# chrism0dwk/covid19uk

Measured on AMD Instinct MI355X. Metric: posterior samples/sec, 380-LAD UK SEIR, higher is better.
Workload: dtype f64; 1 GPU; uk380: M=380 LADs x T=365 days, P=750 parameters; chains_per_gpu=8, chains_total=8, sweep=HMC(16 leapfrogs) + 5 x [S->E move, E->I move, S->E occult, E->I occult], draws_recorded=theta + events[M,T,3] (uint16 counts) + kernel results per sweep, parallelism=chains sharded over 1 GPU(s), no data-path collective

## Files before the change

covid19uk_amd/csrc/handoff.h:

```cpp
#pragma once
#include <hip/hip_runtime.h>

template <typename T> __device__ __forceinline__ T ld_l2(const T *p) { return __hip_atomic_load(p, __ATOMIC_RELAXED, __HIP_MEMORY_SCOPE_AGENT); }
template <typename T, typename V> __device__ __forceinline__ void st_l2(T *p, V v) { __hip_atomic_store(p, v, __ATOMIC_RELAXED, __HIP_MEMORY_SCOPE_AGENT); }
template <typename T, typename V> __device__ __forceinline__ T add_l2(T *p, V v) { return __hip_atomic_fetch_add(p, v, __ATOMIC_RELAXED, __HIP_MEMORY_SCOPE_AGENT); }
template <typename T, typename V> __device__ __forceinline__ T min_l2(T *p, V v) { return __hip_atomic_fetch_min(p, v, __ATOMIC_RELAXED, __HIP_MEMORY_SCOPE_AGENT); }
template <typename T, typename V> __device__ __forceinline__ T max_l2(T *p, V v) { return __hip_atomic_fetch_max(p, v, __ATOMIC_RELAXED, __HIP_MEMORY_SCOPE_AGENT); }

__device__ __forceinline__ bool hs_all(bool ok) { return __builtin_amdgcn_ballot_w64(!ok) == 0ull; }

constexpr int HS_LIMIT = 1 << 22;
constexpr int HS_LIMIT_LEAP = 1 << 21;
constexpr int HS_LIMIT_LL = 1 << 19;
constexpr int HS_LIMIT_ROLES = 4000;
constexpr int HS_CHECK = 256;
constexpr int HS_CHECK_LL = 64;
enum HsCount { HS_CALLER, HS_THREAD0, HS_LANE0, HS_NONE };

template <int SLEEP, int CHECK, int LIMIT, int WHO, int FIRST = SLEEP, int PRIO = -1, typename Ready, typename C = unsigned>
__device__ __forceinline__ bool hs_wait(Ready ready, C *cnt = nullptr, bool backoff = false) {
    static_assert((CHECK & (CHECK - 1)) == 0, "CHECK: a power of two, or 0");
    int spins = 0;
    bool gave_up = false;
    while (!ready()) {
// ... 86 lines not shown
    constexpr int NW = (NDW + 1) / 2;
    const uint4 *pp[1] = {src + min(lane, NW - 1)};
    u32x4 x[1];
    ll_wait<1, 1, HS_CHECK, HS_LIMIT>(pp, seq, late, x);
    if (lane < NW) {
        dst[2 * lane] = (int)x[0].x;
        if (2 * lane + 1 < NDW) dst[2 * lane + 1] = (int)x[0].z;
    }
}

__device__ __forceinline__ void pair_sums_store(uint4 *dst, double th, double cn, unsigned seq) {
    ll_store(dst, th, seq);
    ll_store(dst + 1, cn, seq);
}
__device__ __forceinline__ void pair_sums_wait(const uint4 *src, unsigned seq, unsigned *late, double &th, double &cn) {
    const uint4 *pp[2] = {src, src + 1};
    u32x4 x[2];
    ll_wait<2, 1, HS_CHECK, HS_LIMIT>(pp, seq, late, x);
    th = ll_value(x[0]);
    cn = ll_value(x[1]);
}

__device__ __forceinline__ unsigned pair_token(unsigned sweep, int lidx) { return (sweep * 64u + (unsigned)lidx + 1u) & 0x7fffffffu; }
```

covid19uk_amd/csrc/moves_kernel.h:

```cpp
#pragma once
#include "handoff.h"
#include "sampler_kernels.h"

namespace seir {

#ifdef SEIR_STAMPS
#ifndef SEIR_STAMP_SLOT
#define SEIR_STAMP_SLOT 1
#endif
#define MSTAMP(i) do { if (threadIdx.x == 0 && stamp_on) ((unsigned long long *)(stamp_hs + 16))[i] = __builtin_amdgcn_s_memrealtime(); } while (0)
#else
#define MSTAMP(i) do {} while (0)
#endif

#ifdef PAIR_STAMPS
#define QSTAMP(slot_, step_, i_) do { if (threadIdx.x == 0 && (b_stamp) == 0 && (step_) < 12 && (slot_) < 27) \
    ch.leap_st[((size_t)(slot_) * 12 + (step_)) * 16 + (i_)] = __builtin_amdgcn_s_memrealtime(); } while (0)
#else
#define QSTAMP(slot_, step_, i_) do {} while (0)
#endif

constexpr int MVB = 512;
constexpr int MVW = MVB / WAVE;
constexpr int MVU = 4;
// ... 26 lines not shown

__device__ __forceinline__ void mv_sum2(double &a, double &b2, double *sh) {
    a = wave_sum(a); b2 = wave_sum(b2);
    const int lane = threadIdx.x & 63, wave = threadIdx.x >> 6;
    lds_barrier();
    if (lane == 0) { sh[wave * 2] = a; sh[wave * 2 + 1] = b2; }
    lds_barrier();
    double x = 0.0, y = 0.0;
#pragma unroll
    for (int j = 0; j < MVW; ++j) { x += sh[j * 2]; y += sh[j * 2 + 1]; }
    a = x; b2 = y;
}

struct MvLds {
    const int *rt;
    int *rg;
#ifdef SEIR_STAMPS
    double *stamp_hs; bool stamp_on;
#endif
};

__device__ __forceinline__ double mv_log(double x, const double2 *ltab) { return x == 1.0 ? 0.0 : fast_log(x, ltab); }

__device__ inline void mv_draw(const SamplerCfg &s, const Chains &ch, int b, MoveSpec spec, MvShared &sm, int T) {
    Move &mv = sm.mv;
    const int tid = threadIdx.x;
    if (tid >= 2 * MMAX && tid != 64) return;
    const RngKey key = rng_key(s, ch, b);
    const uint32_t stream = RS_MOVE_BASE + (uint32_t)(spec.scan * 4 + spec.slot);
    if (tid < 2 * MMAX) rng_uniform2(key, stream, (uint32_t)tid, sm.u[tid][0], sm.u[tid][1]);
    if (tid == 64) {
        mv.valid = (s.disable_mask >> (1 + spec.slot)) & 1 ? 0 : 1;
        mv.n = 0; mv.tgt = spec.tgt; mv.kind = spec.kind; mv.slot = spec.slot;
        mv.logq = 0.0; mv.any_dI = 0; mv.LO = T; mv.HI = -1;
        for (int j = 0; j < MMAX; ++j) { mv.tm[j] = mv.tt[j] = mv.tdt[j] = mv.tx[j] = 0; mv.b[j] = -1; sm.pend_valid[j] = -1; }
        double ua, ub;
        rng_uniform2(key, stream, 15u, ua, ub);
        mv.logu = cold_log(ua);
    }
}

__device__ __forceinline__ int wv_popc(unsigned long long m) { return __builtin_popcountll(m); }
__device__ __forceinline__ int wv_kth_bit(unsigned long long mask, int k, int lane) {
    const int below = (int)__builtin_amdgcn_mbcnt_hi((unsigned)(mask >> 32), __builtin_amdgcn_mbcnt_lo((unsigned)mask, 0u));
    const bool me = ((mask >> lane) & 1ull) != 0ull && below == k;
    return (int)__builtin_ctzll(__builtin_amdgcn_ballot_w64(me));
}
constexpr int WV_MCH = 6;
struct HotRows {
    unsigned long long mask[WV_MCH];
    int H;
// ... 568 lines not shown
                *prt += dk;
                if (ra + rb != 0) *prg += ra + rb;
            }
        }
        __syncthreads();
    }
}

__device__ __forceinline__ void mv_trace(const SamplerCfg &s, const Chains &ch, int b, const Move &mv, int acc,
                                         unsigned tr_slot, double lp) {
    if (tr_slot < (unsigned)s.cap) {
        double *tr = ch.tr_mv + (((size_t)tr_slot * s.B + b) * 4 + mv.slot) * NMVTR;
        tr[0] = (double)acc;
        tr[1] = lp;
        for (int j = 0; j < MMAX; ++j) {
            tr[2 + j] = mv.tm[j]; tr[2 + MMAX + j] = mv.tt[j];
            tr[2 + 2 * MMAX + j] = mv.tdt[j]; tr[2 + 3 * MMAX + j] = mv.tx[j];
        }
    }
}

__device__ __forceinline__ void mv_own_rows_to_down(const Dims &d, const Consts &c, const Work &w, int b, const Move &mv,
                                                    double psi, const double2 *ltab, const Move *fp, double *red,
                                                    double *od) {
    double dth = 0.0, dcn = 0.0;
    if (mv.valid && mv.n > 0) own_rows_delta<MVB>(d, c, w, b, mv, psi, 0, d.M, ltab, dth, dcn, fp);
    mv_sum2(dth, dcn, red);
    if (threadIdx.x == 0) {
        od[0] = dth;
        od[1] = dcn;
    }
}

struct PairNote {
    int ok;
    int n, rows[MMAX];
};
static_assert(sizeof(PairNote) == (2 + MMAX) * sizeof(int), "k_move_pair writes the note as 2 + MMAX ints");

__device__ __forceinline__ void move_copy_l2(Move *dst, const Move *src, int t0) {
    const int i = (int)threadIdx.x - t0;
    if (i >= 0 && i < MOVE_DW) reinterpret_cast<int *>(dst)[i] = ld_l2(reinterpret_cast<const int *>(src) + i);
}
__device__ __forceinline__ void wait_token(const unsigned *p_, unsigned token, unsigned *late) {
    hs_wait<1, HS_CHECK, HS_LIMIT, HS_CALLER>([&] { return ld_l2(p_) == token; }, late);
}
__device__ __forceinline__ unsigned wait_token_flag(const unsigned *p_, unsigned token, unsigned *late) {
    unsigned v;
    hs_wait<1, HS_CHECK, HS_LIMIT, HS_CALLER>([&] { return ((v = ld_l2(p_)) & 0x7fffffffu) == token; }, late);
    return v >> 31;
}
static_assert((MOVE_DW + 1) / 2 <= 32, "Chains::llmv holds 32 words per descriptor");
template <bool SOLO, typename TT>
// ... 233 lines not shown
                const int t = t0 + j * WAVE + lane;
                const bool in = t < d.Tp;
                k0[j] = in ? w.K[0][q0 + t] : 0;
                k1[j] = in ? w.K[1][q0 + t] : 0;
                k2[j] = in ? w.K[2][q0 + t] : 0;
            }
#pragma unroll
            for (int j = 0; j < 4; ++j) {
                const int t = t0 + j * WAVE + lane;
                if (t < d.T) {
                    if (s.ev16) {
                        if ((unsigned)(k0[j] | k1[j] | k2[j]) > 0xffffu) ch.ev_overflow[0] = 1u;
                        out16[t * 3 + 0] = (unsigned short)k0[j]; out16[t * 3 + 1] = (unsigned short)k1[j];
                        out16[t * 3 + 2] = (unsigned short)k2[j];
                    } else {
                        out[t * 3 + 0] = k0[j]; out[t * 3 + 1] = k1[j]; out[t * 3 + 2] = k2[j];
                    }
                }
            }
        }
    }
}

template <int NCH, bool SOLO>
__device__ __forceinline__ void pair_step(const Dims &d, const Consts &c, const Work &w, const SamplerCfg &s, const Chains &ch,
                                          MoveSpec se, MoveSpec next, MoveSpec se_next, int have_prev, int have_pre, int pbuf,
                                          int lidx, int dbg, int nband, int nroles, int slot, int b, int fin = 0,
                                          unsigned sweep0 = 0u, int lprev = 0, unsigned tslot = TRACE_NOT_RECORDED) {
    extern __shared__ __attribute__((aligned(16))) int dyn_i[];
    __shared__ MvShared sm_se, sm_nx;
    __shared__ Move pendA, pendB;
    __shared__ PairNote note;
    __shared__ double pre_down[2], s_down[4], s_dsum[2];
    __shared__ double2 ltab[LDSTAB_N];
    __shared__ int s_sel, s_acc_se, s_conf, s_late, s_late2, s_use_pre, s_trans;
    int tid = threadIdx.x;
    asm volatile("" : "+v"(tid));
    asm volatile("" : "+s"(b));
    const int b_stamp = b - d.b0;
    (void)b_stamp;
    QSTAMP(slot, lidx, 0);
    if (slot >= nroles) {
        if (nband == 0) return;
        if (fin) {
            pair_band_finish(d, c, w, s, ch, b, slot - nroles, nband, pair_token(sweep0, lidx), tslot, fin & 2);
            return;
        }
        const unsigned tok = pair_token(ch.sweep[b], lidx);
        const bool r1 = next.kind >= 0 && nroles >= 2, r2 = se_next.kind >= 0 && nroles == 3;
        if ((d.M + nband - 1) / nband > 2 * MVW)
            pair_band_block<SOLO, 4>(d, c, w, s, ch, b, slot - nroles, nband, tok, r1, r2, pbuf ^ 1, slot, lidx);
        else
            pair_band_block<SOLO, 2>(d, c, w, s, ch, b, slot - nroles, nband, tok, r1, r2, pbuf ^ 1, slot, lidx);
        return;
    }
    const int role = slot == nroles - 1 ? 0 : slot + 1;
    const int M = d.M, T = d.T;
    const bool do_se = role == 0 && se.kind >= 0, do_nx = next.kind >= 0, do_pre = se_next.kind >= 0 && nroles == 3;
    if (role == 1 && !do_nx) return;
    if (role == 2 && !do_pre) return;
#ifdef SEIR_STAMPS
    double *stamp_hs = ch.hs + (size_t)b * NHS;
    const bool stamp_on = do_se && b == 0 && se.slot == (SEIR_STAMP_SLOT & 2) && se.scan == 0;
#define PSTAMP(i) do { if (threadIdx.x == 0 && stamp_on) ((unsigned long long *)(stamp_hs + 16))[i] = __builtin_amdgcn_s_memrealtime(); } while (0)
#ifndef SEIR_STAMP_ROLE
#define SEIR_STAMP_ROLE 1
#endif
    const bool rstamp_on = role == SEIR_STAMP_ROLE && b == 0 && se.slot == (SEIR_STAMP_SLOT & 2) && se.scan == 0;
#ifdef SEIR_STAMP_PROPOSE
#define RSTAMP(i) do { if (threadIdx.x == 0 && rstamp_on) ((unsigned long long *)(stamp_hs + 16))[(i) + 4] = __builtin_amdgcn_s_memrealtime(); } while (0)
#undef PSTAMP
#define PSTAMP(i) do {} while (0)
#else
#define RSTAMP(i) do { if (threadIdx.x == 0 && rstamp_on) ((unsigned long long *)(stamp_hs + 16))[i] = __builtin_amdgcn_s_memrealtime(); } while (0)
#endif
#else
#define PSTAMP(i) do {} while (0)
#define RSTAMP(i) do {} while (0)
#endif
    PSTAMP(0);
    RSTAMP(8);
    const bool pre_ok = M <= PRE_RT * MVB;
    const MoveSpec &mine = role == 2 ? se_next : next;
    int pre_se[PRE_RT], pre_nx[PRE_RT];
    mv_prefetch_rows(d, w, s, b, se, do_se && pre_ok, pre_se);
    mv_prefetch_rows(d, w, s, b, mine, (role == 2 || do_nx) && pre_ok, pre_nx);
    const unsigned token = pair_token(ch.sweep[b], lidx);
    double dth0 = 0.0, dcn0 = 0.0;
    int ld_i = 0;
    double ld_d = 0.0;
    if (have_prev) {
        if (tid >= 64 && tid < 64 + MOVE_DW) ld_i = reinterpret_cast<const int *>(ch.mv + (size_t)pbuf * s.B + b)[tid - 64];
        if (tid >= 128 && tid < 128 + MOVE_DW) ld_i = reinterpret_cast<const int *>(ch.mvfix + (size_t)pbuf * s.B + b)[tid - 128];
        if (tid == 192) ld_i = ch.mvsel[(size_t)pbuf * s.B + b];
        if (tid >= 196 && tid < 200) ld_d = ch.Down[(((size_t)pbuf * 2 + ((tid - 196) >> 1)) * s.B + b) * 2 + ((tid - 196) & 1)];
        if (!SOLO) {
            if (tid < s.nrb_d) {
                dth0 = ch.Dpart[((size_t)b * s.nrb_d + tid) * 2];
                dcn0 = ch.Dpart[((size_t)b * s.nrb_d + tid) * 2 + 1];
            }
            for (int i = tid + MVB; i < s.nrb_d; i += MVB) {
                dth0 += ch.Dpart[((size_t)b * s.nrb_d + i) * 2];
                dcn0 += ch.Dpart[((size_t)b * s.nrb_d + i) * 2 + 1];
            }
        }
    }
    constexpr int DW0 = SOLO ? MVB - WAVE : 0;
    if (SOLO && have_prev) {
        static_assert(MVB >= 253, "one thread per band workgroup (plan_sweep: 3 + nband <= 256)");
        const bool few = s.nrb_d <= WAVE;
        const int i0 = few ? tid - DW0 : tid;
        if (few ? tid >= DW0 : (tid & ~(WAVE - 1)) < s.nrb_d) {
            const uint4 *src = ch.llD + (((size_t)pbuf * s.B + b) * s.nrb_d + min(i0, s.nrb_d - 1)) * 2;
            double th, cn;
            pair_sums_wait(src, pair_token(ch.sweep[b], lprev), ch.late + ch.late_fatal + b, th, cn);
            if (i0 < s.nrb_d) { dth0 = th; dcn0 = cn; }
#ifdef PAIR_STAMPS
            if (tid == DW0 && b_stamp == 0 && lidx < 12) ch.leap_st[((size_t)slot * 12 + lidx) * 16 + 7] = __builtin_amdgcn_s_memrealtime();
#endif
        }
    }
    const bool pre_avail = do_se && have_pre;
    if (pre_avail) {
        if (tid >= 256 && tid < 256 + MOVE_DW) ld_i = reinterpret_cast<const int *>(ch.mvs + (size_t)pbuf * s.B + b)[tid - 256];
        if (tid >= 320 && tid < 320 + 2 + MMAX) ld_i = reinterpret_cast<const int *>(ch.prev + (size_t)pbuf * s.B + b)[tid - 320];
        if (tid == 328 || tid == 329) ld_d = ch.DownS[((size_t)pbuf * s.B + b) * 2 + (tid - 328)];
    }
    static_assert(MOVE_DW <= 64 && 2 + MMAX <= 8, "the entry loads of pair_step: disjoint thread ranges");
    double hs_th = 0.0, hs_cn = 0.0, psi = 0.0;
    unsigned tr_slot = 0xffffffffu;
    double2 ld_t = make_double2(0.0, 0.0);
    if (tid < LDSTAB_N) ld_t = c.logtab[tid];
    if (role == 0 && tid == 0) {
        const double *hs = ch.hs + (size_t)b * NHS;
        hs_th = hs[HS_LP_THETA]; hs_cn = hs[HS_LP_CONST];
        tr_slot = SOLO ? tslot : chain_trace_slot(s, ch, ch.sweep[b]);
    }
    psi = w.scal[(size_t)b * NSCAL + SC_PSI];
    QSTAMP(slot, lidx, 6);
    if (do_se && !pre_avail) mv_draw(s, ch, b, se, sm_se, T);
    if (role != 0 || do_nx) mv_draw(s, ch, b, mine, sm_nx, T);
    QSTAMP(slot, lidx, 14);
    if (have_prev) {
        if (tid >= 64 && tid < 64 + MOVE_DW) reinterpret_cast<int *>(&pendA)[tid - 64] = ld_i;
        if (tid >= 128 && tid < 128 + MOVE_DW) reinterpret_cast<int *>(&pendB)[tid - 128] = ld_i;
        if (tid == 192) s_sel = ld_i;
        if (tid >= 196 && tid < 200) s_down[tid - 196] = ld_d;
    }
    if (pre_avail) {
        if (tid >= 256 && tid < 256 + MOVE_DW) reinterpret_cast<int *>(&sm_se.mv)[tid - 256] = ld_i;
        if (tid >= 320 && tid < 320 + 2 + MMAX) reinterpret_cast<int *>(&note)[tid - 320] = ld_i;
        if (tid == 328 || tid == 329) pre_down[tid - 328] = ld_d;
    }
    if (tid < LDSTAB_N) ltab[tid] = ld_t;
    if (have_prev && s.nrb_d <= WAVE && tid >= DW0 && tid < DW0 + WAVE) {
        const double a = wave_sum(dth0), a2 = wave_sum(dcn0);
        if (tid == DW0) { s_dsum[0] = 0.0 + a; s_dsum[1] = 0.0 + a2; }
    }
    if (role != 0) {
        asm volatile("s_waitcnt vmcnt(0)" ::: "memory");
        QSTAMP(slot, lidx, 12);
        __syncthreads();
        QSTAMP(slot, lidx, 13);
        const int late_bit = role == 1 ? 1 : 4, absent_bit = role == 1 ? 2 : 8;
// ... 15 lines not shown
        pendp = &pend;
        if (s.nrb_d <= WAVE) {
            dth0 = s_dsum[0]; dcn0 = s_dsum[1];
        } else {
            mv_sum2(dth0, dcn0, sm_nx.dred);
        }
        dth0 += s_down[s_sel ? 2 : 0];
        dcn0 += s_down[s_sel ? 3 : 1];
        const double ratio = dth0 + dcn0 + pend.logq;
        pend_acc = pend.valid && pend.logu < ratio;
    }
    if (role != 0) {
        const Move *fix = (pend_acc && pendp->tgt == mine.tgt) ? pendp : nullptr;
        RSTAMP(9);
#if defined(SEIR_STAMPS) && defined(SEIR_STAMP_PROPOSE)
        L.stamp_hs = stamp_hs; L.stamp_on = rstamp_on;
#endif
        QSTAMP(slot, lidx, 1);
        mv_rows_to_lds(d, w, s, b, mine, pre_ok, pre_nx, fix, L, rtl);
        mv_propose<NCH>(d, w, s, ch, b, mine, sm_nx, L, ltab);
        QSTAMP(slot, lidx, 2);
        RSTAMP(10);
        Move *out = (role == 1 ? ch.mv : ch.mvs) + (size_t)(pbuf ^ 1) * s.B + b;
        move_copy(out, &sm_nx.mv, MVB - WAVE);
        if (nband > 0 && role == 1 && tid >= MVB - WAVE)
            move_store_ll<MOVE_DW>(ch.llmv + ((size_t)(pbuf ^ 1) * s.B + b) * 32, reinterpret_cast<const int *>(&sm_nx.mv), tid - (MVB - WAVE),
                                   token);
        const Move *fpp = (pend_acc && pendp->any_dI) ? pendp : nullptr;
        double *od = role == 1 ? ch.Down + (((size_t)(pbuf ^ 1) * 2 + 0) * s.B + b) * 2
                               : ch.DownS + ((size_t)(pbuf ^ 1) * s.B + b) * 2;
        mv_own_rows_to_down(d, c, w, b, sm_nx.mv, psi, ltab, fpp, sm_nx.dred, od);
        QSTAMP(slot, lidx, 3);
        RSTAMP(11);
        if (nband > 0) {
            __syncthreads();
            if (tid == 0)
                st_l2(ch.done + (size_t)b * 2 * TAIL_STRIDE + role, token);
        }
        return;
    }
    if (!have_prev && tid == 64) {
        ch.fpend[b].valid = 0;
        if (nband > 0) {
            asm volatile("s_waitcnt vmcnt(0)" ::: "memory");
            st_l2(ch.done + (size_t)b * 2 * TAIL_STRIDE + 4, token);
        }
    }
    bool late = false, late2 = false;
    auto wait_roles = [&]() {
        if (tid == 0) {
            const bool l1 = do_nx && hs_wait<2, 0, HS_LIMIT_ROLES, HS_NONE>([&] { return ld_l2(ch.hand + b) == token; });
            const bool l2 = do_pre && hs_wait<2, 0, HS_LIMIT_ROLES, HS_NONE>([&] { return ld_l2(ch.hand2 + b) == token; });
            s_late = l1; s_late2 = l2;
            if (l1 || l2) ch.late[b] += 1;
// ... 33 lines not shown
            st_l2(ch.done + (size_t)b * 2 * TAIL_STRIDE + 5, token);
    }
    bool se_acc = false;
    if (do_se) {
        const Move *fpp = (pend_acc && pendp->any_dI) ? pendp : nullptr;
        if (tid == 0) {
            int use = pre_avail && note.ok;
            if (use) {
                const Move &mv = sm_se.mv;
                for (int i = 0; i < mv.n; ++i) {
                    for (int j = 0; j < note.n; ++j) use &= mv.m[i] != note.rows[j];
                    if (pend_acc)
                        for (int j = 0; j < pendp->n; ++j) use &= mv.m[i] != pendp->m[j];
                }
            }
            s_use_pre = use;
        }
        lds_barrier();
        const bool use_pre = s_use_pre != 0;
        double dth = 0.0, dcn = 0.0;
        if (!use_pre) {
            if (pre_avail) {
                lds_barrier();
                mv_draw(s, ch, b, se, sm_se, T);
            }
            mv_rows_to_lds(d, w, s, b, se, pre_ok, pre_se, nullptr, L, rtl);
            PSTAMP(2);
            mv_propose<NCH>(d, w, s, ch, b, se, sm_se, L, ltab);
            PSTAMP(3);
        }
        const Move &mv = sm_se.mv;
        if (use_pre && fpp == nullptr) {
            dth = pre_down[0]; dcn = pre_down[1];
        } else {
            if (mv.valid && mv.n > 0) own_rows_delta<MVB>(d, c, w, b, mv, psi, 0, M, ltab, dth, dcn, fpp);
            PSTAMP(4);
            mv_sum2(dth, dcn, sm_se.dred);
        }
        if (tid == 0) {
            const double ratio = dth + dcn + mv.logq;
            s_acc_se = (mv.valid && mv.logu < ratio) ? 1 : 0;
        }
        lds_barrier();
        se_acc = s_acc_se != 0;
        if (se_acc && !waited) { wait_roles(); waited = true; }
        if (tid == 0) s_trans = 0;
        if (se_acc) mv_apply_rows(d, w, s, b, mv, &s_trans);
// ... 39 lines not shown
            move_copy(ch.mvfix + (size_t)(pbuf ^ 1) * s.B + b, &sm_nx.mv, MVB - WAVE);
            const Move *fpp = (pend_acc && pendp->any_dI) ? pendp : nullptr;
            mv_own_rows_to_down(d, c, w, b, sm_nx.mv, psi, ltab, fpp, sm_nx.dred,
                                ch.Down + (((size_t)(pbuf ^ 1) * 2 + 1) * s.B + b) * 2);
        }
        PSTAMP(7);
        QSTAMP(slot, lidx, 3);
    }
    if (do_pre && tid == 0) {
        int *nt = reinterpret_cast<int *>(ch.prev + (size_t)(pbuf ^ 1) * s.B + b);
        const int n_pend = pend_acc ? pendp->n : 0, n_se = se_acc ? sm_se.mv.n : 0;
        const bool se_keeps = !se_acc || (((s_trans & (se_next.kind == 0 ? 1 : 2)) == 0) && n_pend + n_se <= MMAX);
        nt[0] = (se_keeps && !(waited && late2)) ? 1 : 0;
        nt[1] = n_pend + (se_keeps ? n_se : 0);
#pragma unroll
        for (int j = 0; j < MMAX; ++j) {
            int row = -1;
            if (j < n_pend) row = pendp->m[j];
            else if (se_keeps && j - n_pend < n_se) row = sm_se.mv.m[j - n_pend];
            nt[2 + j] = row;
        }
    }
    if (nband > 0) {
        __syncthreads();
        if (tid == 0)
            st_l2(ch.done + (size_t)b * 2 * TAIL_STRIDE + 0, token | ((do_nx && s_conf) ? 0x80000000u : 0u));
    }
}

template <int NCH>
__global__ __launch_bounds__(MVB) void k_move_pair(Dims d, Consts c, Work w, SamplerCfg s, Chains ch, MoveSpec se,
                                                   MoveSpec next, MoveSpec se_next, int have_prev, int have_pre,
                                                   int pbuf, int nbk, int lidx, int dbg, int nband) {
    debug_skew(d);
    const int nroles = (int)gridDim.x / nbk - nband, slot = (int)blockIdx.x / nbk;
    const int b = d.b0 + (int)blockIdx.x - slot * nbk;
    if (d.nlive > 0 && (int)blockIdx.x - slot * nbk >= d.nlive) return;
    pair_step<NCH, false>(d, c, w, s, ch, se, next, se_next, have_prev, have_pre, pbuf, lidx, dbg, nband, nroles, slot, b);
    const int b_stamp = b - d.b0;
    (void)b_stamp;
    QSTAMP(slot, lidx, 8);
}

constexpr int PBAR_STRIDE = 64;
__device__ __forceinline__ void pair_chain_barrier(const Chains &ch, int b, unsigned target, int b_stamp = 0, int st_slot = 0,
                                                   int st_step = 0) {
    asm volatile("s_waitcnt vmcnt(0)" ::: "memory");
    __syncthreads();
    QSTAMP(st_slot, st_step, 10);
    if (threadIdx.x == 0) {
        unsigned *cnt = ch.pbar + (size_t)b * PBAR_STRIDE;
        const unsigned old = add_l2(cnt, 1u);
        __builtin_amdgcn_fence(__ATOMIC_ACQUIRE, "agent");
#ifndef PBAR_SLEEP
#define PBAR_SLEEP 1
#endif
        if (old + 1u != target)
            hs_wait<PBAR_SLEEP, HS_CHECK, HS_LIMIT, HS_CALLER>([&] { return (int)(ld_l2(cnt) - target) >= 0; }, ch.late + ch.late_fatal + b);
        asm volatile("s_waitcnt vmcnt(0)" ::: "memory");
    }
    QSTAMP(st_slot, st_step, 11);
    __syncthreads();
}

__device__ __forceinline__ void pair_band_next_step() {
    __syncthreads();
    if (threadIdx.x == 0) {
        __builtin_amdgcn_fence(__ATOMIC_ACQUIRE, "agent");
        asm volatile("s_waitcnt vmcnt(0)" ::: "memory");
    }
    __syncthreads();
}

constexpr int PAIR_DBG_DELAYS = 16 | 32 | 64 | 128;
__device__ __forceinline__ void pair_debug_delay(int dbg, int slot, int nroles, int pair, int b) {
    const bool band = slot >= nroles, role0 = slot == nroles - 1;
    bool on = ((dbg & 16) && band) || ((dbg & 32) && role0) || ((dbg & 64) && !band && !role0);
    if (dbg & 128) {
        unsigned h = (unsigned)slot * 0x9e3779b1u ^ (unsigned)pair * 0x85ebca6bu ^ (unsigned)b * 0xc2b2ae35u;
        h ^= h >> 15; h *= 0x2c1b3c6du; h ^= h >> 12;
        on = on || h % 3u == 0u;
    }
    if (on)
        for (int i = 0; i < 9; ++i) __builtin_amdgcn_s_sleep(127);
}

template <int NCH>
__global__ __launch_bounds__(MVB) void k_move_pairs(Dims d, Consts c, Work w, SamplerCfg s, Chains ch, int npairs, int pre_on,
                                                    int nbk, int dbg, int nband, unsigned pbase, int fin) {
    debug_skew(d);
    const int nroles = (int)gridDim.x / nbk - nband, slot = (int)blockIdx.x / nbk;
    const int b = d.b0 + (int)blockIdx.x - slot * nbk;
    if (d.nlive > 0 && (int)blockIdx.x - slot * nbk >= d.nlive) return;
    const MoveSpec none{-1, 0, 0, 0};
    const unsigned sweep0 = ch.sweep[b];
    const unsigned tslot = chain_trace_slot(s, ch, sweep0);
    for (int pair = 0; pair <= npairs; ++pair) {
        const bool closing = pair == npairs;
        const int scan = pair >> 1, half = pair & 1, nh = half ^ 1, nscan = scan + half;
        const bool pre = pre_on && pair + 1 < npairs;
        const MoveSpec se = closing ? none : MoveSpec{half, 0, 2 * half, scan};
        const MoveSpec nx = closing ? MoveSpec{-2, 0, 0, 0} : MoveSpec{half, 1, 2 * half + 1, scan};
        const MoveSpec se_next = pre ? MoveSpec{nh, 0, 2 * nh, nscan} : none;
        if (dbg & PAIR_DBG_DELAYS) pair_debug_delay(dbg, slot, nroles, pair, b);
        pair_step<NCH, true>(d, c, w, s, ch, se, nx, se_next, pair > 0 ? 1 : 0, (pair > 0 && pre_on && !closing) ? 1 : 0, pair & 1,
                       closing ? 62 : pair, closing ? 0 : dbg, (closing && !fin) ? 0 : nband, nroles, slot, b, closing ? fin : 0, sweep0,
                       pair - 1, tslot);
        if (closing) break;
        const int b_stamp = b - d.b0;
        (void)b_stamp;
        QSTAMP(slot, pair, 8);
        if (slot < nroles) pair_chain_barrier(ch, b, pbase + (unsigned)((pair + 1) * nroles), b_stamp, slot, pair);
        else pair_band_next_step();
        QSTAMP(slot, pair, 9);
    }
}

inline size_t k_move_pa2_lds_bytes(const Dims &d) {
    return sizeof(int) * ((size_t)2 * d.M);
}
inline size_t k_move_pairs_lds_bytes(const Dims &d) {
    const size_t need = k_move_pa2_lds_bytes(d), half = 82 * 1024;
    return need > half ? need : half;
}

}
```

covid19uk_amd/csrc/sampler_kernels.h:

```cpp
#pragma once
#include "handoff.h"
#include "logprob_kernels.h"
#include "philox.h"
#include "trace_slot.h"

namespace seir {

constexpr int MMAX = 4;
constexpr int NHS = 32;
enum {
    HS_EPS = 0,
    HS_LP_THETA,
    HS_LP_CONST,
    HS_LP0,
    HS_K0,
    HS_DA_ERR, HS_DA_STEP, HS_DA_LOGAVG, HS_DA_MU,
    HS_RV_N,
    HS_ACC,
    HS_LOGACC
};

struct SamplerCfg {
    int B, dmax, nmax, mmax, occult_nmax, n_scans, tr_lo, tr_hi, L;
    uint32_t k0, k1;
// ... 22 lines not shown

constexpr int MOVE_DW = (int)(sizeof(Move) / 4);
static_assert(sizeof(Move) % 4 == 0 && MOVE_DW <= 64, "Move must fit one dword per lane of a wave");
__device__ __forceinline__ void move_copy(Move *dst, const Move *src, int t0) {
    const int i = (int)threadIdx.x - t0;
    if (i >= 0 && i < MOVE_DW) reinterpret_cast<int *>(dst)[i] = reinterpret_cast<const int *>(src)[i];
}

constexpr int TAIL_STRIDE = 16;
constexpr int ROLE_SLOTS = 64;
constexpr int NMVTR = 2 + 4 * MMAX;

struct PairNote;
struct Chains {
    double *q, *p, *q0, *grad, *var, *rv_mean, *rv_m2;
    double *hs;
    Move *mv;
    Move *fpend;
    Move *mvfix;
    unsigned *hand;
    unsigned *late;
    int late_fatal;
    double *finpart;
    unsigned *pbar;
    unsigned *done;
    unsigned long long *tail;
    unsigned long long *leap;
    double *k0part;
    double *irl0;
    unsigned long long *leap_st;
    uint4 *llK;
    uint4 *llR;
    uint4 *llP;
    uint4 *llTS;
    uint4 *llT;
    uint4 *llmv;
    uint4 *llD;
    unsigned *hand2;
    Move *mvs;
    double *DownS;
    struct PairNote *prev;
    int *mvsel;
    double *Dpart;
    double *Down;
    unsigned *sweep;
    unsigned *slot0;
    double *tr_theta;
// ... 2321 lines not shown
```

covid19uk_amd/csrc/seir_hip.hip:

```cpp
#include <hip/hip_runtime.h>

#include <algorithm>
#include <atomic>
#include <cmath>
#include <cstdarg>
#include <cstdio>
#include <cstring>
#include <new>
#include <vector>

#include "../../include/seir_hip.h"
#include "sampler_kernels.h"
#include "sim_kernels.h"
#include "moves_kernel.h"
#include "rt_kernels.h"
#include "sweep_plan.h"

using namespace seir;

static_assert(plan::WAVE == WAVE && plan::CT_MAXC == CT_MAXC && plan::ROLE_SLOTS == ROLE_SLOTS,
              "sweep_plan.h reads the kernels' constants");

static thread_local char g_err[512] = "";

// ... 920 lines not shown
    Chains ch{};
    int record_events = 1;
    int cus = 0, leap_occ[2] = {0, 0};
    bool pairs_lds_attr = false;
    std::vector<void *> allocs;
    int ngroups = 1;
    std::vector<hipStream_t> gstream;
    std::vector<hipGraph_t> graph;
    std::vector<hipGraphExec_t> gexec;
    hipEvent_t ev_fork = nullptr;
    std::vector<hipEvent_t> ev_join;
    hipStream_t copy_stream = nullptr;
    hipEvent_t ev_burst = nullptr, ev_copy = nullptr;
    bool copy_pending = false;
    bool use_graph = false;
    int leap_rows = 0;
    std::vector<hipEvent_t> prof_ev;
    int prof_i = -1;
    bool vt_dirty = true;
    unsigned long long leap_rsteps = 0;
    unsigned long long leap_steps = 0;
    bool xcd_local = false;
    unsigned long long tail_count = 0;
    unsigned pbar_count = 0;
    int pair_debug = 0;
    int moves_mode = 0;
    int graph_skew = 0, graph_aff = 3;
    bool have_state = false;
    double *ev_stage = nullptr;
    enum { R_OTHER = 0, R_STATE = 1, R_HANDOFF = 2 };
    struct Region { void *p; size_t bytes; int kind; };
    std::vector<Region> regions;
    void *snap[2] = {nullptr, nullptr};
    bool snap_valid[2] = {false, false};
    size_t snap_bytes = 0;
    bool poisoned = false;
    int poison_chain = 0;
    unsigned poison_count = 0;
    int hmc_mode = 0;
    int thin_pending = 1;
};

template <typename T>
static int s_alloc(seir_sampler *s, T **p, size_t count, int kind = seir_sampler::R_OTHER) {
    void *q = nullptr;
    const size_t bytes = (count ? count : 1) * sizeof(T);
    HIP_TRY(hipMalloc(&q, bytes));
// ... 136 lines not shown
    S_STATE(ch.q, (size_t)B * d.Pp); S_STATE(ch.p, (size_t)B * d.Pp); S_STATE(ch.q0, (size_t)B * d.Pp);
    S_STATE(ch.grad, (size_t)B * d.Pp); S_STATE(ch.var, (size_t)B * d.Pp);
    S_STATE(ch.rv_mean, (size_t)B * d.Pp); S_STATE(ch.rv_m2, (size_t)B * d.Pp);
    S_STATE(ch.hs, (size_t)B * NHS);
    S_HAND(ch.mv, (size_t)2 * B);
    S_HAND(ch.fpend, (size_t)B);
    S_HAND(ch.mvfix, (size_t)2 * B);
    S_HAND(ch.mvsel, (size_t)2 * B);
    S_HAND(ch.hand, (size_t)B);
    S_HAND(ch.late, (size_t)2 * B);
    ch.late_fatal = B;
    S_HAND(ch.tail, (size_t)B * TAIL_STRIDE + (size_t)B * TAIL_FLAG_STRIDE);
    S_HAND(ch.leap, (size_t)B * LEAP_CH);
    S_HAND(ch.llK, (size_t)B * 2 * (d.Mp / 16) * d.Tp);
    S_HAND(ch.llR, (size_t)B * 2 * d.ntc * d.Mp);
    S_HAND(ch.llP, (size_t)B * 2 * d.ntc * (d.Mp / 16));
    S_HAND(ch.llTS, (size_t)B * 2 * d.ntc * (d.Mp / 16) * 4);
    S_HAND(ch.llT, (size_t)B * ((size_t)d.Tp + 2 * (size_t)d.Mp + 8));
    S_HAND(ch.llmv, (size_t)2 * B * 32);
    S_HAND(ch.k0part, (size_t)B * ROLE_SLOTS);
    S_HAND(ch.irl0, (size_t)B);
    S_ALLOC(ch.leap_st, (size_t)(B + 2) * 16 * 8 + 4096);
    S_HAND(ch.done, (size_t)B * 2 * TAIL_STRIDE);
    S_HAND(ch.pbar, (size_t)B * PBAR_STRIDE);
    S_HAND(ch.finpart, (size_t)B * ROLE_SLOTS * 4);
    S_HAND(ch.hand2, (size_t)B);
    S_HAND(ch.mvs, (size_t)2 * B);
    S_HAND(ch.DownS, (size_t)2 * B * 2);
    S_HAND(ch.prev, (size_t)2 * B);
    S_HAND(ch.Dpart, (size_t)B * c.nrb_d * 2);
    S_HAND(ch.llD, (size_t)2 * B * c.nrb_d * 2);
    S_HAND(ch.Down, (size_t)2 * 2 * B * 2);
    S_STATE(ch.sweep, (size_t)B); S_STATE(ch.slot0, 1);
    S_ALLOC(ch.tr_theta, (size_t)c.cap * B * d.P);
    {
        char *tre = nullptr;
        S_ALLOC(tre, s->record_events ? (size_t)c.cap * B * d.M * d.T * 3 * (c.ev16 ? 2 : 4) : 4);
        ch.tr_events = tre;
    }
    S_ALLOC(ch.ev_overflow, 1);
    S_ALLOC(ch.tr_hmc, (size_t)c.cap * B * 3);
    S_ALLOC(ch.tr_mv, (size_t)c.cap * B * 4 * NMVTR);
    S_ALLOC(s->ev_stage, (size_t)B * d.M * d.T * 3);
#undef S_STATE
#undef S_HAND
    if (!rc) {
        const size_t Bm = (size_t)ctx->Bmax;
// ... 40 lines not shown
        const size_t plds = k_move_pa2_lds_bytes(d);
        for (const void *fn : {(const void *)move_pair_fn(nch), (const void *)move_pa2_fn(nch)})
            if (plds > 64 * 1024) (void)hipFuncSetAttribute(fn, hipFuncAttributeMaxDynamicSharedMemorySize, (int)plds);
    }
    if (rc) { seir_sampler_destroy(s); return rc; }
    *out = s;
    return 0;
}

extern "C" int seir_sampler_xcd_local(seir_sampler *s) { return (s && s->xcd_local) ? 1 : 0; }

static int sampler_check(seir_sampler *s) {
    if (!s) return fail(SEIR_ERR_INVALID, "null sampler");
    HIP_TRY(hipSetDevice(s->ctx->device));
    return 0;
}

static int reset_handoffs(seir_sampler *s) {
    hipStream_t st = s->ctx->stream;
    for (const auto &r : s->regions)
        if (r.kind == seir_sampler::R_HANDOFF) HIP_TRY(hipMemsetAsync(r.p, 0, r.bytes, st));
    s->leap_rsteps = s->leap_steps = 0;
    s->tail_count = 0;
    s->pbar_count = 0;
    s->poisoned = false;
    return 0;
}

extern "C" int seir_sampler_set_launch_form(seir_sampler *s, int32_t hmc_mode, int32_t moves_mode) {
    int rc = sampler_check(s);
    if (rc) return rc;
    if (moves_mode < 0 || moves_mode > 4 || hmc_mode < 0 || hmc_mode > 6)
        return fail(SEIR_ERR_INVALID, "moves_mode is 0..4, hmc_mode 0..6");
    if (hmc_mode != s->hmc_mode || moves_form(moves_mode, s->cfg.n_scans) != s->moves_mode) {
        HIP_TRY(hipStreamSynchronize(s->ctx->stream));
        drop_graph(s);
        apply_launch_form(s, hmc_mode, moves_mode);
    }
    return 0;
}

extern "C" int seir_sampler_launch_form(seir_sampler *s, int32_t *hmc_mode, int32_t *moves_mode) {
    if (!s) return fail(SEIR_ERR_INVALID, "null sampler");
    if (hmc_mode) *hmc_mode = s->hmc_mode;
    if (moves_mode) *moves_mode = s->moves_mode;
    return 0;
}
// ... 409 lines not shown
        const auto pa2_fn = move_pa2_fn(p.nch);
        for (int scan = 0; scan < c.n_scans; ++scan)
            for (int slot = 0; slot < 4; ++slot) {
                const MoveSpec spec{slot >= 2 ? 1 : 0, slot & 1, slot, scan};
                hipLaunchKernelGGL(pa2_fn, gm, dim3(MVB), plds, st, d, ctx->c, ctx->w, c, s->ch, spec,
                                   have_prev, pbuf);
                pbuf ^= 1;
                hipLaunchKernelGGL((k_move_delta<true>), gm, dim3(DELTA_THREADS), 0, st, d, ctx->c, ctx->w, c, s->ch, pbuf, 0);
                have_prev = 1;
            }
        if (have_prev) {
            const MoveSpec none{-2, 0, 0, 0};
            hipLaunchKernelGGL(pa2_fn, gm, dim3(MVB), plds, st, d, ctx->c, ctx->w, c, s->ch, none, 1, pbuf);
        }
    } else {
        const int npairs = 2 * c.n_scans;
        const auto pair_fn = move_pair_fn(p.nch);
        Dims dp = d;
        dp.nlive = p.pair_nlive;
        SamplerCfg cp = c;
        if (p.nband) cp.nrb_d = p.nband;
        if (p.moves == SweepPlan::PAIRS) {
            hipLaunchKernelGGL(move_pairs_fn(p.nch), dim3((3 + p.nband) * p.nbk), dim3(MVB), k_move_pairs_lds_bytes(d), st, dp, ctx->c, ctx->w, cp,
                               s->ch, npairs, 1, p.nbk, s->pair_debug, p.nband, s->pbar_count, s->record_events ? 3 : 1);
            s->pbar_count += (unsigned)(npairs * 3);
        } else {
            int have_pre = 0;
            for (int scan = 0; scan < c.n_scans; ++scan)
                for (int half = 0; half < 2; ++half) {
                    const int pair = 2 * scan + half;
                    const MoveSpec se{half, 0, 2 * half, scan}, nx{half, 1, 2 * half + 1, scan};
                    const bool pre = p.pre && pair + 1 < npairs;
                    const int nh = (half + 1) & 1, nscan = scan + (half == 1 ? 1 : 0);
                    const MoveSpec se_next = pre ? MoveSpec{nh, 0, 2 * nh, nscan} : MoveSpec{-1, 0, 0, 0};
                    hipLaunchKernelGGL(pair_fn, dim3(((pre ? 3 : 2) + p.nband) * p.nbk), dim3(MVB), plds, st, dp, ctx->c, ctx->w, cp,
                                       s->ch, se, nx, se_next, have_prev, have_pre, pbuf, p.nbk, pair, s->pair_debug, p.nband);
                    have_pre = pre ? 1 : 0;
                    pbuf ^= 1;
                    if (!p.nband)
                        hipLaunchKernelGGL((k_move_delta<false>), gm, dim3(DELTA_THREADS), 0, st, d, ctx->c, ctx->w, c, s->ch, pbuf, 1);
                    have_prev = 1;
                }
            if (have_prev) {
                const MoveSpec none{-1, 0, 0, 0}, close{-2, 0, 0, 0};
                hipLaunchKernelGGL(pair_fn, dim3(nb), dim3(MVB), plds, st, d, ctx->c, ctx->w, cp, s->ch, none, close, none, 1,
                                   0, pbuf, nb, 62, 0, 0);
                if (p.fpend == SweepPlan::F_APPLY) hipLaunchKernelGGL(k_apply_fpend, gm, dim3(256), 0, st, d, ctx->c, ctx->w, c, s->ch);
            }
// ... 262 lines not shown
```

Before: 27980 posterior samples/sec.

## Replace per-pair counting barrier with token-based role handoff in persistent move kernel

Removes the shared atomic counter barrier that made all role blocks of a chain wait for each other after every move pair. Each role now publishes a per-role token and waits only on the specific upstream roles it depends on, using a parity-indexed 'last' word. Role 1 also keeps its own move, selection and down-sums in shared memory so it does not reload them from global memory. The sweep index comes from a kernel-start value rather than repeated global reads. This lets roles run ahead and cuts barrier and reload latency, at the cost of more intricate ordering logic with possible race or deadlock risk.

After: 27800 posterior samples/sec. Within noise of the previous version (-0.6%).

```diff
diff --git a/covid19uk_amd/csrc/handoff.h b/covid19uk_amd/csrc/handoff.h
--- a/covid19uk_amd/csrc/handoff.h
+++ b/covid19uk_amd/csrc/handoff.h
@@ -132,3 +132,17 @@
 }
 
 __device__ __forceinline__ unsigned pair_token(unsigned sweep, int lidx) { return (sweep * 64u + (unsigned)lidx + 1u) & 0x7fffffffu; }
+
+template <int WHO = HS_CALLER>
+__device__ __forceinline__ unsigned pair_roles_wait(const unsigned *last, const unsigned *r1, const unsigned *r2, unsigned token,
+                                                    unsigned *late) {
+    unsigned flag = 0u;
+    hs_wait<1, HS_CHECK, HS_LIMIT, WHO>([&] {
+        const unsigned a = last != nullptr ? ld_l2(last) : token;
+        const unsigned x = r1 != nullptr ? ld_l2(r1) : token;
+        const unsigned y = r2 != nullptr ? ld_l2(r2) : token;
+        flag = a >> 31;
+        return (a & 0x7fffffffu) == token && (int)((x - token) << 1) >= 0 && (int)((y - token) << 1) >= 0;
+    }, late);
+    return flag;
+}
diff --git a/covid19uk_amd/csrc/moves_kernel.h b/covid19uk_amd/csrc/moves_kernel.h
--- a/covid19uk_amd/csrc/moves_kernel.h
+++ b/covid19uk_amd/csrc/moves_kernel.h
@@ -72,11 +72,12 @@
 
 __device__ __forceinline__ double mv_log(double x, const double2 *ltab) { return x == 1.0 ? 0.0 : fast_log(x, ltab); }
 
-__device__ inline void mv_draw(const SamplerCfg &s, const Chains &ch, int b, MoveSpec spec, MvShared &sm, int T) {
+__device__ inline void mv_draw(const SamplerCfg &s, const Chains &ch, int b, MoveSpec spec, MvShared &sm, int T,
+                               const unsigned *sweep = nullptr) {
     Move &mv = sm.mv;
     const int tid = threadIdx.x;
     if (tid >= 2 * MMAX && tid != 64) return;
-    const RngKey key = rng_key(s, ch, b);
+    const RngKey key{s.k0, s.k1, (uint32_t)(s.chain0 + b), sweep != nullptr ? *sweep : ch.sweep[b]};
     const uint32_t stream = RS_MOVE_BASE + (uint32_t)(spec.scan * 4 + spec.slot);
     if (tid < 2 * MMAX) rng_uniform2(key, stream, (uint32_t)tid, sm.u[tid][0], sm.u[tid][1]);
     if (tid == 64) {
@@ -691,13 +692,14 @@
 
 __device__ __forceinline__ void mv_own_rows_to_down(const Dims &d, const Consts &c, const Work &w, int b, const Move &mv,
                                                     double psi, const double2 *ltab, const Move *fp, double *red,
-                                                    double *od) {
+                                                    double *od, double *keep = nullptr) {
     double dth = 0.0, dcn = 0.0;
     if (mv.valid && mv.n > 0) own_rows_delta<MVB>(d, c, w, b, mv, psi, 0, d.M, ltab, dth, dcn, fp);
     mv_sum2(dth, dcn, red);
     if (threadIdx.x == 0) {
         od[0] = dth;
         od[1] = dcn;
+        if (keep != nullptr) { keep[0] = dth; keep[1] = dcn; }
     }
 }
 
@@ -977,16 +979,27 @@
     }
 }
 
+__device__ __forceinline__ unsigned pair_debug_hash(int slot, int pair, int b) {
+    unsigned h = (unsigned)slot * 0x9e3779b1u ^ (unsigned)pair * 0x85ebca6bu ^ (unsigned)b * 0xc2b2ae35u;
+    h ^= h >> 15; h *= 0x2c1b3c6du; h ^= h >> 12;
+    return h;
+}
+__device__ __forceinline__ int role_of(int slot, int nroles) { return slot == nroles - 1 ? 0 : slot + 1; }
+constexpr int PAIR_LAST = 6;
+constexpr int PAIR_LEFT = 8;
+static_assert(PAIR_LEFT + 2 < 2 * TAIL_STRIDE, "Chains::done: 2 TAIL_STRIDE words per chain");
+
 template <int NCH, bool SOLO>
 __device__ __forceinline__ void pair_step(const Dims &d, const Consts &c, const Work &w, const SamplerCfg &s, const Chains &ch,
                                           MoveSpec se, MoveSpec next, MoveSpec se_next, int have_prev, int have_pre, int pbuf,
                                           int lidx, int dbg, int nband, int nroles, int slot, int b, int fin = 0,
-                                          unsigned sweep0 = 0u, int lprev = 0, unsigned tslot = TRACE_NOT_RECORDED) {
+                                          unsigned sweep0 = 0u, int lprev = 0, unsigned tslot = TRACE_NOT_RECORDED,
+                                          int sel_in = -1) {
     extern __shared__ __attribute__((aligned(16))) int dyn_i[];
     __shared__ MvShared sm_se, sm_nx;
     __shared__ Move pendA, pendB;
     __shared__ PairNote note;
-    __shared__ double pre_down[2], s_down[4], s_dsum[2];
+    __shared__ double pre_down[2], s_down[4], s_dsum[2], own_down[2];
     __shared__ double2 ltab[LDSTAB_N];
     __shared__ int s_sel, s_acc_se, s_conf, s_late, s_late2, s_use_pre, s_trans;
     int tid = threadIdx.x;
@@ -1001,7 +1014,7 @@
             pair_band_finish(d, c, w, s, ch, b, slot - nroles, nband, pair_token(sweep0, lidx), tslot, fin & 2);
             return;
         }
-        const unsigned tok = pair_token(ch.sweep[b], lidx);
+        const unsigned tok = pair_token(SOLO ? sweep0 : ch.sweep[b], lidx);
         const bool r1 = next.kind >= 0 && nroles >= 2, r2 = se_next.kind >= 0 && nroles == 3;
         if ((d.M + nband - 1) / nband > 2 * MVW)
             pair_band_block<SOLO, 4>(d, c, w, s, ch, b, slot - nroles, nband, tok, r1, r2, pbuf ^ 1, slot, lidx);
@@ -1009,7 +1022,7 @@
             pair_band_block<SOLO, 2>(d, c, w, s, ch, b, slot - nroles, nband, tok, r1, r2, pbuf ^ 1, slot, lidx);
         return;
     }
-    const int role = slot == nroles - 1 ? 0 : slot + 1;
+    const int role = role_of(slot, nroles);
     const int M = d.M, T = d.T;
     const bool do_se = role == 0 && se.kind >= 0, do_nx = next.kind >= 0, do_pre = se_next.kind >= 0 && nroles == 3;
     if (role == 1 && !do_nx) return;
@@ -1040,15 +1053,29 @@
     int pre_se[PRE_RT], pre_nx[PRE_RT];
     mv_prefetch_rows(d, w, s, b, se, do_se && pre_ok, pre_se);
     mv_prefetch_rows(d, w, s, b, mine, (role == 2 || do_nx) && pre_ok, pre_nx);
-    const unsigned token = pair_token(ch.sweep[b], lidx);
+    const unsigned sweep_now = SOLO ? sweep0 : ch.sweep[b];
+    const unsigned token = pair_token(sweep_now, lidx);
+    const unsigned *sweep_p = SOLO ? &sweep_now : nullptr;
     double dth0 = 0.0, dcn0 = 0.0;
     int ld_i = 0;
     double ld_d = 0.0;
+    const bool own = SOLO && role_of(slot, nroles) == 1 && have_prev && sel_in >= 0;
+    if (own) {
+        if (tid >= 64 && tid < 64 + MOVE_DW) ld_i = reinterpret_cast<const int *>(&sm_nx.mv)[tid - 64];
+        if (tid == 192) ld_i = sel_in;
+        if (tid >= 196 && tid < 198) ld_d = own_down[tid - 196];
+        if (sel_in) {
+            if (tid >= 128 && tid < 128 + MOVE_DW) ld_i = reinterpret_cast<const int *>(ch.mvfix + (size_t)pbuf * s.B + b)[tid - 128];
+            if (tid >= 198 && tid < 200) ld_d = ch.Down[(((size_t)pbuf * 2 + 1) * s.B + b) * 2 + (tid - 198)];
+        }
+    }
     if (have_prev) {
-        if (tid >= 64 && tid < 64 + MOVE_DW) ld_i = reinterpret_cast<const int *>(ch.mv + (size_t)pbuf * s.B + b)[tid - 64];
-        if (tid >= 128 && tid < 128 + MOVE_DW) ld_i = reinterpret_cast<const int *>(ch.mvfix + (size_t)pbuf * s.B + b)[tid - 128];
-        if (tid == 192) ld_i = ch.mvsel[(size_t)pbuf * s.B + b];
-        if (tid >= 196 && tid < 200) ld_d = ch.Down[(((size_t)pbuf * 2 + ((tid - 196) >> 1)) * s.B + b) * 2 + ((tid - 196) & 1)];
+        if (!own) {
+            if (tid >= 64 && tid < 64 + MOVE_DW) ld_i = reinterpret_cast<const int *>(ch.mv + (size_t)pbuf * s.B + b)[tid - 64];
+            if (tid >= 128 && tid < 128 + MOVE_DW) ld_i = reinterpret_cast<const int *>(ch.mvfix + (size_t)pbuf * s.B + b)[tid - 128];
+            if (tid == 192) ld_i = ch.mvsel[(size_t)pbuf * s.B + b];
+            if (tid >= 196 && tid < 200) ld_d = ch.Down[(((size_t)pbuf * 2 + ((tid - 196) >> 1)) * s.B + b) * 2 + ((tid - 196) & 1)];
+        }
         if (!SOLO) {
             if (tid < s.nrb_d) {
                 dth0 = ch.Dpart[((size_t)b * s.nrb_d + tid) * 2];
@@ -1068,7 +1095,7 @@
         if (few ? tid >= DW0 : (tid & ~(WAVE - 1)) < s.nrb_d) {
             const uint4 *src = ch.llD + (((size_t)pbuf * s.B + b) * s.nrb_d + min(i0, s.nrb_d - 1)) * 2;
             double th, cn;
-            pair_sums_wait(src, pair_token(ch.sweep[b], lprev), ch.late + ch.late_fatal + b, th, cn);
+            pair_sums_wait(src, pair_token(sweep_now, lprev), ch.late + ch.late_fatal + b, th, cn);
             if (i0 < s.nrb_d) { dth0 = th; dcn0 = cn; }
 #ifdef PAIR_STAMPS
             if (tid == DW0 && b_stamp == 0 && lidx < 12) ch.leap_st[((size_t)slot * 12 + lidx) * 16 + 7] = __builtin_amdgcn_s_memrealtime();
@@ -1093,8 +1120,8 @@
     }
     psi = w.scal[(size_t)b * NSCAL + SC_PSI];
     QSTAMP(slot, lidx, 6);
-    if (do_se && !pre_avail) mv_draw(s, ch, b, se, sm_se, T);
-    if (role != 0 || do_nx) mv_draw(s, ch, b, mine, sm_nx, T);
+    if (do_se && !pre_avail) mv_draw(s, ch, b, se, sm_se, T, sweep_p);
+    if (role != 0 || do_nx) mv_draw(s, ch, b, mine, sm_nx, T, sweep_p);
     QSTAMP(slot, lidx, 14);
     if (have_prev) {
         if (tid >= 64 && tid < 64 + MOVE_DW) reinterpret_cast<int *>(&pendA)[tid - 64] = ld_i;
@@ -1156,6 +1183,9 @@
         QSTAMP(slot, lidx, 2);
         RSTAMP(10);
         Move *out = (role == 1 ? ch.mv : ch.mvs) + (size_t)(pbuf ^ 1) * s.B + b;
+        if (SOLO && role == 1 && have_pre && tid >= MVB - WAVE)
+            pair_roles_wait<HS_LANE0>(nullptr, nullptr, ch.done + (size_t)b * 2 * TAIL_STRIDE + PAIR_LEFT + 2, pair_token(sweep_now, lprev),
+                                      ch.late + ch.late_fatal + b);
         move_copy(out, &sm_nx.mv, MVB - WAVE);
         if (nband > 0 && role == 1 && tid >= MVB - WAVE)
             move_store_ll<MOVE_DW>(ch.llmv + ((size_t)(pbuf ^ 1) * s.B + b) * 32, reinterpret_cast<const int *>(&sm_nx.mv), tid - (MVB - WAVE),
@@ -1163,7 +1193,7 @@
         const Move *fpp = (pend_acc && pendp->any_dI) ? pendp : nullptr;
         double *od = role == 1 ? ch.Down + (((size_t)(pbuf ^ 1) * 2 + 0) * s.B + b) * 2
                                : ch.DownS + ((size_t)(pbuf ^ 1) * s.B + b) * 2;
-        mv_own_rows_to_down(d, c, w, b, sm_nx.mv, psi, ltab, fpp, sm_nx.dred, od);
+        mv_own_rows_to_down(d, c, w, b, sm_nx.mv, psi, ltab, fpp, sm_nx.dred, od, (SOLO && role == 1) ? own_down : nullptr);
         QSTAMP(slot, lidx, 3);
         RSTAMP(11);
         if (nband > 0) {
@@ -1243,7 +1273,7 @@
         if (!use_pre) {
             if (pre_avail) {
                 lds_barrier();
-                mv_draw(s, ch, b, se, sm_se, T);
+                mv_draw(s, ch, b, se, sm_se, T, sweep_p);
             }
             mv_rows_to_lds(d, w, s, b, se, pre_ok, pre_se, nullptr, L, rtl);
             PSTAMP(2);
@@ -1329,9 +1359,13 @@
         }
     }
     if (nband > 0) {
+        if (SOLO) asm volatile("s_waitcnt vmcnt(0)" ::: "memory");
         __syncthreads();
-        if (tid == 0)
-            st_l2(ch.done + (size_t)b * 2 * TAIL_STRIDE + 0, token | ((do_nx && s_conf) ? 0x80000000u : 0u));
+        if (tid == 0) {
+            const unsigned last = token | ((do_nx && s_conf) ? 0x80000000u : 0u);
+            st_l2(ch.done + (size_t)b * 2 * TAIL_STRIDE + 0, last);
+            if (SOLO) st_l2(ch.done + (size_t)b * 2 * TAIL_STRIDE + PAIR_LAST + (pbuf & 1), last);
+        }
     }
 }
 
@@ -1349,25 +1383,25 @@
     QSTAMP(slot, lidx, 8);
 }
 
-constexpr int PBAR_STRIDE = 64;
-__device__ __forceinline__ void pair_chain_barrier(const Chains &ch, int b, unsigned target, int b_stamp = 0, int st_slot = 0,
-                                                   int st_step = 0) {
+__device__ __forceinline__ int pair_role_next_step(const Chains &ch, int b, int role, unsigned token, int par, bool r1, bool r2,
+                                                   int dbg, int b_stamp = 0, int st_slot = 0, int st_step = 0) {
+    __shared__ int s_flag;
     asm volatile("s_waitcnt vmcnt(0)" ::: "memory");
     __syncthreads();
     QSTAMP(st_slot, st_step, 10);
     if (threadIdx.x == 0) {
-        unsigned *cnt = ch.pbar + (size_t)b * PBAR_STRIDE;
-        const unsigned old = add_l2(cnt, 1u);
+        unsigned *done = ch.done + (size_t)b * 2 * TAIL_STRIDE;
+        if (role != 0) st_l2(done + PAIR_LEFT + role, token);
+        if ((dbg & 1024) && pair_debug_hash(st_slot + 101, st_step, b) % 3u == 0u)
+            for (int i = 0; i < 9; ++i) __builtin_amdgcn_s_sleep(127);
+        s_flag = (int)pair_roles_wait(role != 0 ? done + PAIR_LAST + par : nullptr, (role != 1 && r1) ? done + PAIR_LEFT + 1 : nullptr,
+                                      (role == 0 && r2) ? done + PAIR_LEFT + 2 : nullptr, token, ch.late + ch.late_fatal + b);
+        QSTAMP(st_slot, st_step, 11);
         __builtin_amdgcn_fence(__ATOMIC_ACQUIRE, "agent");
-#ifndef PBAR_SLEEP
-#define PBAR_SLEEP 1
-#endif
-        if (old + 1u != target)
-            hs_wait<PBAR_SLEEP, HS_CHECK, HS_LIMIT, HS_CALLER>([&] { return (int)(ld_l2(cnt) - target) >= 0; }, ch.late + ch.late_fatal + b);
         asm volatile("s_waitcnt vmcnt(0)" ::: "memory");
     }
-    QSTAMP(st_slot, st_step, 11);
     __syncthreads();
+    return s_flag;
 }
 
 __device__ __forceinline__ void pair_band_next_step() {
@@ -1379,22 +1413,19 @@
     __syncthreads();
 }
 
-constexpr int PAIR_DBG_DELAYS = 16 | 32 | 64 | 128;
+constexpr int PAIR_DBG_DELAYS = 16 | 32 | 64 | 128 | 256 | 512;
 __device__ __forceinline__ void pair_debug_delay(int dbg, int slot, int nroles, int pair, int b) {
     const bool band = slot >= nroles, role0 = slot == nroles - 1;
     bool on = ((dbg & 16) && band) || ((dbg & 32) && role0) || ((dbg & 64) && !band && !role0);
-    if (dbg & 128) {
-        unsigned h = (unsigned)slot * 0x9e3779b1u ^ (unsigned)pair * 0x85ebca6bu ^ (unsigned)b * 0xc2b2ae35u;
-        h ^= h >> 15; h *= 0x2c1b3c6du; h ^= h >> 12;
-        on = on || h % 3u == 0u;
-    }
+    on = on || ((dbg & 256) && !band && role_of(slot, nroles) == 1) || ((dbg & 512) && !band && role_of(slot, nroles) == 2);
+    if (dbg & 128) on = on || pair_debug_hash(slot, pair, b) % 3u == 0u;
     if (on)
         for (int i = 0; i < 9; ++i) __builtin_amdgcn_s_sleep(127);
 }
 
 template <int NCH>
 __global__ __launch_bounds__(MVB) void k_move_pairs(Dims d, Consts c, Work w, SamplerCfg s, Chains ch, int npairs, int pre_on,
-                                                    int nbk, int dbg, int nband, unsigned pbase, int fin) {
+                                                    int nbk, int dbg, int nband, int fin) {
     debug_skew(d);
     const int nroles = (int)gridDim.x / nbk - nband, slot = (int)blockIdx.x / nbk;
     const int b = d.b0 + (int)blockIdx.x - slot * nbk;
@@ -1402,6 +1433,7 @@
     const MoveSpec none{-1, 0, 0, 0};
     const unsigned sweep0 = ch.sweep[b];
     const unsigned tslot = chain_trace_slot(s, ch, sweep0);
+    int sel = -1;
     for (int pair = 0; pair <= npairs; ++pair) {
         const bool closing = pair == npairs;
         const int scan = pair >> 1, half = pair & 1, nh = half ^ 1, nscan = scan + half;
@@ -1412,12 +1444,13 @@
         if (dbg & PAIR_DBG_DELAYS) pair_debug_delay(dbg, slot, nroles, pair, b);
         pair_step<NCH, true>(d, c, w, s, ch, se, nx, se_next, pair > 0 ? 1 : 0, (pair > 0 && pre_on && !closing) ? 1 : 0, pair & 1,
                        closing ? 62 : pair, closing ? 0 : dbg, (closing && !fin) ? 0 : nband, nroles, slot, b, closing ? fin : 0, sweep0,
-                       pair - 1, tslot);
+                       pair - 1, tslot, sel);
         if (closing) break;
         const int b_stamp = b - d.b0;
         (void)b_stamp;
         QSTAMP(slot, pair, 8);
-        if (slot < nroles) pair_chain_barrier(ch, b, pbase + (unsigned)((pair + 1) * nroles), b_stamp, slot, pair);
+        if (slot < nroles)
+            sel = pair_role_next_step(ch, b, role_of(slot, nroles), pair_token(sweep0, pair), pair & 1, true, pre, dbg, b_stamp, slot, pair);
         else pair_band_next_step();
         QSTAMP(slot, pair, 9);
     }
diff --git a/covid19uk_amd/csrc/sampler_kernels.h b/covid19uk_amd/csrc/sampler_kernels.h
--- a/covid19uk_amd/csrc/sampler_kernels.h
+++ b/covid19uk_amd/csrc/sampler_kernels.h
@@ -68,7 +68,6 @@
     unsigned *late;
     int late_fatal;
     double *finpart;
-    unsigned *pbar;
     unsigned *done;
     unsigned long long *tail;
     unsigned long long *leap;
diff --git a/covid19uk_amd/csrc/seir_hip.hip b/covid19uk_amd/csrc/seir_hip.hip
--- a/covid19uk_amd/csrc/seir_hip.hip
+++ b/covid19uk_amd/csrc/seir_hip.hip
@@ -966,7 +966,6 @@
     unsigned long long leap_steps = 0;
     bool xcd_local = false;
     unsigned long long tail_count = 0;
-    unsigned pbar_count = 0;
     int pair_debug = 0;
     int moves_mode = 0;
     int graph_skew = 0, graph_aff = 3;
@@ -1149,7 +1148,6 @@
     S_HAND(ch.irl0, (size_t)B);
     S_ALLOC(ch.leap_st, (size_t)(B + 2) * 16 * 8 + 4096);
     S_HAND(ch.done, (size_t)B * 2 * TAIL_STRIDE);
-    S_HAND(ch.pbar, (size_t)B * PBAR_STRIDE);
     S_HAND(ch.finpart, (size_t)B * ROLE_SLOTS * 4);
     S_HAND(ch.hand2, (size_t)B);
     S_HAND(ch.mvs, (size_t)2 * B);
@@ -1236,7 +1234,6 @@
         if (r.kind == seir_sampler::R_HANDOFF) HIP_TRY(hipMemsetAsync(r.p, 0, r.bytes, st));
     s->leap_rsteps = s->leap_steps = 0;
     s->tail_count = 0;
-    s->pbar_count = 0;
     s->poisoned = false;
     return 0;
 }
@@ -1692,8 +1689,7 @@
         if (p.nband) cp.nrb_d = p.nband;
         if (p.moves == SweepPlan::PAIRS) {
             hipLaunchKernelGGL(move_pairs_fn(p.nch), dim3((3 + p.nband) * p.nbk), dim3(MVB), k_move_pairs_lds_bytes(d), st, dp, ctx->c, ctx->w, cp,
-                               s->ch, npairs, 1, p.nbk, s->pair_debug, p.nband, s->pbar_count, s->record_events ? 3 : 1);
-            s->pbar_count += (unsigned)(npairs * 3);
+                               s->ch, npairs, 1, p.nbk, s->pair_debug, p.nband, s->record_events ? 3 : 1);
         } else {
             int have_pre = 0;
             for (int scan = 0; scan < c.n_scans; ++scan)
```
